# thuanz123/enhancing-transformers

Measured on AMD Instinct MI355X. Metric: images/sec ViT-VQGAN-base 256px stage-1 train; VQ argmin match-rate, higher is better.
Workload: dtype fp16; 1 GPU; imagenet_vitvq_base.yaml AE training step (1 fwd + 1 bwd + grad all-reduce + AdamW), loss = 1.0*L2 + 1.0*codebook (LPIPS/GAN weights 0), K=8192 x 32 l2-normalised codes, fp32 master weights, fp16 MFMA operands / fp32 accumulate, dynamic loss scale (now 65536; device-side inf/nan step skip + GradScaler update rule); per_gpu_batch=128, global_batch=128, image=256x256, parallelism=dp1, hip_graph_replay=False

## Files before the change

### enhancing-transformers_amd/csrc/common.h

```cpp
#pragma once
#include <hip/hip_runtime.h>
#include <stdint.h>
#include <stdio.h>
#include "../../include/enh_hip.h"

#define LDS_AS __attribute__((address_space(3)))
#define GLB_AS __attribute__((address_space(1)))
#ifdef ENH_GLDS_AUX_OVERRIDE
#define ENH_GLDS_AUX ENH_GLDS_AUX_OVERRIDE
#else
#define ENH_GLDS_AUX 0
#endif

typedef __attribute__((ext_vector_type(4))) float f32x4;
typedef __attribute__((ext_vector_type(4))) unsigned int u32x4;
typedef __attribute__((ext_vector_type(2))) unsigned int u32x2;
typedef __attribute__((ext_vector_type(16))) float f32x16;
typedef __attribute__((ext_vector_type(8))) __bf16 bf16x8;
typedef __attribute__((ext_vector_type(8))) short s16x8;
typedef __attribute__((ext_vector_type(4))) short s16x4;
typedef __attribute__((__vector_size__(4 * sizeof(__bf16)))) __bf16 bf16x4_t;

void enh_set_error(const char* fmt, ...);
int enh_check_launch(const char* what);
// ... 79 lines not shown
#define ENH_DT_DISPATCH(dtype, CALL)                    \
  do {                                                   \
    if ((dtype) == ENH_DT_F16) { typedef F16 OT; CALL; } \
    else { typedef BF16 OT; CALL; }                      \
  } while (0)
#define ENH_REQUIRE_DT(dtype, what) ENH_REQUIRE((dtype) == ENH_DT_BF16 || (dtype) == ENH_DT_F16, ENH_E_BADARG, what ": dtype must be ENH_DT_BF16 (0) or ENH_DT_F16 (1), got %d", (int)(dtype))

__device__ __forceinline__ float tanh_x3(float x) {
  const float x2 = x * x;
  const float t = __builtin_amdgcn_exp2f(x * 2.8853900817779268f);
  const float big = 1.f - 2.f * __builtin_amdgcn_rcpf(t + 1.f);
  const float small = x * (1.f + x2 * (-0.33333333333f + x2 * (0.13333333333f + x2 * -0.05396825397f)));
  return x2 < 0.0144f ? small : big;
}

__device__ inline s16x4 lds_tr_read_b64(const void* lds_ptr) {
  bf16x4_t v = __builtin_amdgcn_ds_read_tr16_b64_v4bf16((LDS_AS bf16x4_t*)lds_ptr);
  return __builtin_bit_cast(s16x4, v);
}

__device__ inline void lds_tr_read_b64_asm(unsigned long long& out, const void* lds_ptr) {
  const unsigned addr = (unsigned)(uintptr_t)(LDS_AS const void*)lds_ptr;
  asm volatile("ds_read_b64_tr_b16 %0, %1" : "=v"(out) : "v"(addr) : "memory");
}

__device__ inline float wave_sum(float v) {
#pragma unroll
  for (int o = 32; o > 0; o >>= 1) v += __shfl_xor(v, o, 64);
  return v;
}
__device__ inline float wave_max(float v) {
#pragma unroll
  for (int o = 32; o > 0; o >>= 1) v = fmaxf(v, __shfl_xor(v, o, 64));
  return v;
}

template <int NW, typename T>
__device__ __forceinline__ void block_publish(T wave_value, T* s_w) {
  static_assert(NW == 4 || NW == 16, "workgroups of 256 or 1024 threads");
  __syncthreads();
  if ((threadIdx.x & 63) == 0) s_w[threadIdx.x >> 6] = wave_value;
  __syncthreads();
}
template <int NW>
__device__ __forceinline__ float block_sum(float v, float* s_w) {
  block_publish<NW>(wave_sum(v), s_w);
  if constexpr (NW == 4) return ((s_w[0] + s_w[1]) + s_w[2]) + s_w[3];
  float s = 0.f;
#pragma unroll
  for (int i = 0; i < NW; ++i) s += s_w[i];
  return s;
}
template <int NW>
__device__ __forceinline__ float block_max(float v, float* s_w) {
  block_publish<NW>(wave_max(v), s_w);
  if constexpr (NW == 4) return fmaxf(fmaxf(s_w[0], s_w[1]), fmaxf(s_w[2], s_w[3]));
  float s = s_w[0];
#pragma unroll
  for (int i = 1; i < NW; ++i) s = fmaxf(s, s_w[i]);
  return s;
}
template <int NW>
__device__ __forceinline__ int block_count(int v, int* s_w) {
#pragma unroll
  for (int o = 32; o > 0; o >>= 1) v += __shfl_xor(v, o, 64);
  block_publish<NW>(v, s_w);
  int s = 0;
#pragma unroll
  for (int i = 0; i < NW; ++i) s += s_w[i];
  return s;
}

__device__ __forceinline__ u32x4 philox4x32_10(uint32_t k0, uint32_t k1, u32x4 c) {
#pragma unroll
  for (int r = 0; r < 10; ++r) {
    const uint32_t h0 = __umulhi(0xD2511F53u, c.x), l0 = 0xD2511F53u * c.x;
    const uint32_t h1 = __umulhi(0xCD9E8D57u, c.z), l1 = 0xCD9E8D57u * c.z;
    c = u32x4{h1 ^ c.y ^ k0, l1, h0 ^ c.w ^ k1, l0};
    k0 += 0x9E3779B9u; k1 += 0xBB67AE85u;
  }
  return c;
}

__device__ inline float fixed_order_rowsum16(const float* __restrict__ part, int rows, int64_t stride, int64_t n, bool n_ok, float* s_red ) {
  const int col = threadIdx.x & 15, grp = threadIdx.x >> 4;
  const int per = (rows + 15) / 16;
  const int r0 = grp * per, r1 = r0 + per < rows ? r0 + per : rows;
  float a = 0.f;
  if (n_ok)
    for (int r = r0; r < r1; ++r) a += part[(int64_t)r * stride + n];
  s_red[grp * 16 + col] = a;
  __syncthreads();
  float t = 0.f;
  if (grp == 0)
    for (int g = 0; g < 16; ++g) t += s_red[g * 16 + col];
  return t;
}
```

### enhancing-transformers_amd/csrc/elementwise.hip

```cpp
#include "common.h"

template <typename OT>
__global__ void patchify_kernel(const float* __restrict__ img, int B, int C, int H, int W, int p,
                                uint16_t* __restrict__ out, int64_t total4) {
  const int64_t i = (int64_t)blockIdx.x * blockDim.x + threadIdx.x;
  if (i >= total4) return;
  const int p4 = p >> 2, gx_n = W / p, gy_n = H / p;
  int64_t r = i;
  const int q = (int)(r % p4); r /= p4;
  const int ph = (int)(r % p); r /= p;
  const int c = (int)(r % C); r /= C;
  const int gx = (int)(r % gx_n);
  const int gy = (int)((r / gx_n) % gy_n);
  const int b = (int)(r / ((int64_t)gx_n * gy_n));
  const float4 v = *reinterpret_cast<const float4*>(img + (((size_t)b * C + c) * H + (size_t)gy * p + ph) * W + (size_t)gx * p + q * 4);
  *reinterpret_cast<uint2*>(out + (size_t)i * 4) = make_uint2(pack2<OT>(v.x, v.y), pack2<OT>(v.z, v.w));
}

template <typename OT>
__global__ __launch_bounds__(256) void unpatchify_loss_kernel(
    const float* __restrict__ pix, const float* __restrict__ target, int B, int C, int H, int W, int p, float w_l1,
    float w_l2, float inv_numel, float* __restrict__ xrec, double* __restrict__ sums, uint16_t* __restrict__ dpix,
    int64_t total4, const float* __restrict__ gscale) {
  __shared__ float s_l1[4], s_l2[4];
  if (gscale) inv_numel *= *gscale;
  const int64_t i = (int64_t)blockIdx.x * blockDim.x + threadIdx.x;
  float l1 = 0.f, l2 = 0.f;
  if (i < total4) {
    const int p4 = p >> 2, gx_n = W / p, gy_n = H / p;
    int64_t r = i;
    const int q = (int)(r % p4); r /= p4;
    const int ph = (int)(r % p); r /= p;
    const int c = (int)(r % C); r /= C;
    const int gx = (int)(r % gx_n);
    const int gy = (int)((r / gx_n) % gy_n);
    const int b = (int)(r / ((int64_t)gx_n * gy_n));
    const size_t off = (((size_t)b * C + c) * H + (size_t)gy * p + ph) * W + (size_t)gx * p + q * 4;
    const float4 v = *reinterpret_cast<const float4*>(pix + (size_t)i * 4);
    if (xrec) *reinterpret_cast<float4*>(xrec + off) = v;
    if (target) {
      const float4 x = *reinterpret_cast<const float4*>(target + off);
      const float d[4] = {v.x - x.x, v.y - x.y, v.z - x.z, v.w - x.w};
      float g[4];
#pragma unroll
      for (int k = 0; k < 4; ++k) {
        l1 += fabsf(d[k]);
        l2 += d[k] * d[k];
        const float sg = d[k] > 0.f ? 1.f : (d[k] < 0.f ? -1.f : 0.f);
        g[k] = (w_l1 * sg + w_l2 * 2.f * d[k]) * inv_numel;
      }
      if (dpix) *reinterpret_cast<uint2*>(dpix + (size_t)i * 4) = make_uint2(pack2<OT>(g[0], g[1]), pack2<OT>(g[2], g[3]));
    }
  }
  if (sums) {
    l1 = wave_sum(l1);
    l2 = wave_sum(l2);
    if ((threadIdx.x & 63) == 0) { s_l1[threadIdx.x >> 6] = l1; s_l2[threadIdx.x >> 6] = l2; }
    __syncthreads();
    if (threadIdx.x == 0) {
      atomicAdd(&sums[0], (double)((s_l1[0] + s_l1[1]) + (s_l1[2] + s_l1[3])));
      atomicAdd(&sums[1], (double)((s_l2[0] + s_l2[1]) + (s_l2[2] + s_l2[3])));
    }
  }
}

template <typename OT>
__global__ __launch_bounds__(256) void colsum_h16_kernel(const uint16_t* __restrict__ x, int64_t M, int64_t N,
                                                          int64_t ldx, int64_t rows_per_block, float* __restrict__ out, int64_t part_stride) {
  __shared__ float s_part[3][128];
  const int lane = threadIdx.x & 63, wave = threadIdx.x >> 6;
  const int64_t n0 = (int64_t)blockIdx.x * 128 + lane * 2;
  const int64_t m_begin = (int64_t)blockIdx.y * rows_per_block;
  int64_t m_end = m_begin + rows_per_block;
  if (m_end > M) m_end = M;
  float a0 = 0.f, a1 = 0.f;
  if (n0 < N) {
    for (int64_t m = m_begin + wave; m < m_end; m += 4) {
      const uint32_t u = *reinterpret_cast<const uint32_t*>(x + (size_t)m * ldx + n0);
      a0 += unpack_lo<OT>(u);
      a1 += unpack_hi<OT>(u);
    }
  }
  if (wave > 0) { s_part[wave - 1][lane * 2] = a0; s_part[wave - 1][lane * 2 + 1] = a1; }
  __syncthreads();
  if (wave == 0 && n0 < N) {
    for (int ww = 0; ww < 3; ++ww) { a0 += s_part[ww][lane * 2]; a1 += s_part[ww][lane * 2 + 1]; }
    { if (part_stride) out[(int64_t)blockIdx.y * part_stride + n0] = a0; else atomicAdd(&out[n0], a0); }
    { if (part_stride) out[(int64_t)blockIdx.y * part_stride + n0 + 1] = a1; else atomicAdd(&out[n0 + 1], a1); }
  }
}

template <typename OT>
__global__ __launch_bounds__(256) void colsum_h16_wide_kernel(const uint16_t* __restrict__ x, int64_t M, int64_t N, int64_t ldx,
                                                               int64_t rows_per_block, float* __restrict__ out, int64_t part_stride) {
  __shared__ float s_part[3][512];
  const int lane = threadIdx.x & 63, wave = threadIdx.x >> 6;
  const int64_t n0 = (int64_t)blockIdx.x * 512 + lane * 8;
  const int64_t m_begin = (int64_t)blockIdx.y * rows_per_block;
  int64_t m_end = m_begin + rows_per_block;
  if (m_end > M) m_end = M;
  float acc[8] = {0.f, 0.f, 0.f, 0.f, 0.f, 0.f, 0.f, 0.f};
  if (n0 < N) {
    const uint16_t* col = x + n0;
    int64_t m = m_begin + wave;
    for (; m + 12 < m_end; m += 16) {
      u32x4 v[4];
#pragma unroll
      for (int r = 0; r < 4; ++r) v[r] = *reinterpret_cast<const u32x4*>(col + (size_t)(m + 4 * r) * ldx);
#pragma unroll
      for (int r = 0; r < 4; ++r)
#pragma unroll
        for (int k = 0; k < 4; ++k) {
          acc[2 * k] += unpack_lo<OT>(v[r][k]);
          acc[2 * k + 1] += unpack_hi<OT>(v[r][k]);
        }
    }
    for (; m < m_end; m += 4) {
      const u32x4 v = *reinterpret_cast<const u32x4*>(col + (size_t)m * ldx);
#pragma unroll
      for (int k = 0; k < 4; ++k) {
        acc[2 * k] += unpack_lo<OT>(v[k]);
        acc[2 * k + 1] += unpack_hi<OT>(v[k]);
      }
    }
  }
  if (wave > 0) {
#pragma unroll
    for (int k = 0; k < 8; ++k) s_part[wave - 1][lane * 8 + k] = acc[k];
  }
  __syncthreads();
  if (wave == 0 && n0 < N) {
#pragma unroll
    for (int k = 0; k < 8; ++k) {
      float a = acc[k];
      for (int ww = 0; ww < 3; ++ww) a += s_part[ww][lane * 8 + k];
      { if (part_stride) out[(int64_t)blockIdx.y * part_stride + n0 + k] = a; else atomicAdd(&out[n0 + k], a); }
    }
  }
}

template <typename OT>
__global__ void cast_f32_h16_kernel(const float* __restrict__ x, uint16_t* __restrict__ y, int64_t n) {
  const int64_t i = ((int64_t)blockIdx.x * blockDim.x + threadIdx.x) * 4;
  if (i + 3 < n) {
    const float4 v = *reinterpret_cast<const float4*>(x + i);
    *reinterpret_cast<uint2*>(y + i) = make_uint2(pack2<OT>(v.x, v.y), pack2<OT>(v.z, v.w));
  } else {
    for (int64_t k = i; k < n; ++k) y[k] = pack1<OT>(x[k]);
  }
}

template <typename OT, bool CLIP>
__global__ void adamw_kernel(float* __restrict__ p, const float* __restrict__ g, float* __restrict__ m,
                             float* __restrict__ v, uint16_t* __restrict__ p16, int64_t n, float lr, float beta1,
                             float beta2, float eps, float wd, float gscale, float inv_bc1, float inv_sqrt_bc2, const float* __restrict__ skip,
                             const float* __restrict__ loss_scale, const float* __restrict__ clip_coef, float clip_value) {
  const int64_t i = ((int64_t)blockIdx.x * blockDim.x + threadIdx.x) * 4;
  if (i >= n) return;
  if (skip && *skip != 0.f) return;
  if (loss_scale) gscale /= *loss_scale;
  if (CLIP && clip_coef) gscale *= *clip_coef;
  float pv[4], gv[4], mv[4], vv[4];
  const bool full = i + 3 < n;
  if (full) {
    const float4 a = *reinterpret_cast<const float4*>(p + i), b = *reinterpret_cast<const float4*>(g + i);
    const float4 c = *reinterpret_cast<const float4*>(m + i), d = *reinterpret_cast<const float4*>(v + i);
    pv[0] = a.x; pv[1] = a.y; pv[2] = a.z; pv[3] = a.w; gv[0] = b.x; gv[1] = b.y; gv[2] = b.z; gv[3] = b.w;
    mv[0] = c.x; mv[1] = c.y; mv[2] = c.z; mv[3] = c.w; vv[0] = d.x; vv[1] = d.y; vv[2] = d.z; vv[3] = d.w;
  } else {
    for (int k = 0; k < 4; ++k) {
      const bool ok = i + k < n;
      pv[k] = ok ? p[i + k] : 0.f; gv[k] = ok ? g[i + k] : 0.f; mv[k] = ok ? m[i + k] : 0.f; vv[k] = ok ? v[i + k] : 0.f;
    }
  }
#pragma unroll
  for (int k = 0; k < 4; ++k) {
    float gg = gv[k] * gscale;
    if (CLIP && clip_value > 0.f) gg = gg > clip_value ? clip_value : (gg < -clip_value ? -clip_value : gg);
    pv[k] = pv[k] * (1.0f - lr * wd);
    mv[k] = mv[k] * beta1 + gg * (1.0f - beta1);
    vv[k] = vv[k] * beta2 + gg * gg * (1.0f - beta2);
    const float denom = sqrtf(vv[k]) * inv_sqrt_bc2 + eps;
    pv[k] = pv[k] - (lr * inv_bc1) * (mv[k] / denom);
  }
  if (full) {
    *reinterpret_cast<float4*>(p + i) = make_float4(pv[0], pv[1], pv[2], pv[3]);
    *reinterpret_cast<float4*>(m + i) = make_float4(mv[0], mv[1], mv[2], mv[3]);
    *reinterpret_cast<float4*>(v + i) = make_float4(vv[0], vv[1], vv[2], vv[3]);
    if (p16) *reinterpret_cast<uint2*>(p16 + i) = make_uint2(pack2<OT>(pv[0], pv[1]), pack2<OT>(pv[2], pv[3]));
  } else {
    for (int k = 0; k < 4 && i + k < n; ++k) {
      p[i + k] = pv[k]; m[i + k] = mv[k]; v[i + k] = vv[k];
      if (p16) p16[i + k] = pack1<OT>(pv[k]);
    }
  }
}

extern "C" int enh_patchify(const float* img, int B, int C, int H, int W, int p, enh_h16* patches, int dtype, void* stream) {
  ENH_REQUIRE_DT(dtype, "enh_patchify");
  ENH_REQUIRE(img && patches, ENH_E_BADARG, "enh_patchify: null pointer");
  ENH_REQUIRE(B > 0 && C > 0 && p > 0 && p % 4 == 0 && H % p == 0 && W % p == 0, ENH_E_SHAPE, "enh_patchify: need p %% 4 == 0 and H,W divisible by p (B=%d C=%d H=%d W=%d p=%d)", B, C, H, W, p);
  const int64_t total4 = (int64_t)B * C * H * W / 4;
  ENH_DT_DISPATCH(dtype, (patchify_kernel<OT><<<(int)((total4 + 255) / 256), 256, 0, (hipStream_t)stream>>>(img, B, C, H, W, p, patches, total4)));
  return enh_check_launch("enh_patchify");
}

extern "C" int enh_unpatchify_loss(const float* pix, const float* target, int B, int C, int H, int W, int p, float w_l1,
                                   float w_l2, float* xrec, double* sums, enh_h16* dpix_bf16, const float* grad_scale_dev, int dtype, void* stream) {
  ENH_REQUIRE_DT(dtype, "enh_unpatchify_loss");
  ENH_REQUIRE(pix && (xrec || target), ENH_E_BADARG, "enh_unpatchify_loss: null pointer");
  ENH_REQUIRE(B > 0 && C > 0 && p > 0 && p % 4 == 0 && H % p == 0 && W % p == 0, ENH_E_SHAPE, "enh_unpatchify_loss: need p %% 4 == 0 and H,W divisible by p");
  const int64_t numel = (int64_t)B * C * H * W, total4 = numel / 4;
  ENH_DT_DISPATCH(dtype, (unpatchify_loss_kernel<OT><<<(int)((total4 + 255) / 256), 256, 0, (hipStream_t)stream>>>(
      pix, target, B, C, H, W, p, w_l1, w_l2, 1.0f / (float)numel, xrec, target ? sums : nullptr, dpix_bf16, total4, grad_scale_dev)));
  return enh_check_launch("enh_unpatchify_loss");
}

__global__ __launch_bounds__(256) void colsum_reduce_kernel(const float* __restrict__ part, int chunks, int64_t N, float* __restrict__ out, int accumulate) {
  __shared__ float s_red[256];
  const int64_t n = (int64_t)blockIdx.x * 16 + (threadIdx.x & 15);
  const float t = fixed_order_rowsum16(part, chunks, N, n, n < N, s_red);
  if ((threadIdx.x >> 4) == 0 && n < N) out[n] = accumulate ? out[n] + t : t;
}

int enh_colsum_reduce_launch(const float* part, int chunks, int64_t N, float* out, int accumulate, hipStream_t s) {
  colsum_reduce_kernel<<<dim3((unsigned)((N + 15) / 16)), 256, 0, s>>>(part, chunks, N, out, accumulate);
  return enh_check_launch("colsum_reduce");
}

static int64_t colsum_chunks(int64_t M) {
  const int64_t chunks = (M + 511) / 512;
  return chunks > 256 ? 256 : chunks;
}

extern "C" size_t enh_colsum_h16_workspace_bytes(int64_t M, int64_t N) { return M > 0 && N > 0 ? (size_t)colsum_chunks(M) * N * sizeof(float) : 0; }

static int colsum_h16_impl(const enh_h16* x, int64_t M, int64_t N, int64_t ldx, float* out, int accumulate, float* part, int dtype, void* stream) {
  ENH_REQUIRE_DT(dtype, "enh_colsum_h16");
  ENH_REQUIRE(x && out, ENH_E_BADARG, "enh_colsum_h16: null pointer");
  ENH_REQUIRE(M > 0 && N > 0 && N % 2 == 0 && ldx % 2 == 0, ENH_E_SHAPE, "enh_colsum_h16: N and ldx must be even");
  hipStream_t s = (hipStream_t)stream;
  if (!accumulate && !part) {
    const int rc = enh_zero_f32_launch(out, N, s);
    if (rc) return rc;
  }
  const int64_t chunks = colsum_chunks(M);
  const int64_t rows_per_block = (M + chunks - 1) / chunks;
  float* dst = part ? part : out;
  const int64_t stride = part ? N : 0;
  if (N % 8 == 0 && ldx % 8 == 0 && ((uintptr_t)x & 15) == 0) {
    dim3 grid((unsigned)((N + 511) / 512), (unsigned)chunks);
    ENH_DT_DISPATCH(dtype, (colsum_h16_wide_kernel<OT><<<grid, 256, 0, s>>>(x, M, N, ldx, rows_per_block, dst, stride)));
  } else {
    dim3 grid((unsigned)((N + 127) / 128), (unsigned)chunks);
    ENH_DT_DISPATCH(dtype, (colsum_h16_kernel<OT><<<grid, 256, 0, s>>>(x, M, N, ldx, rows_per_block, dst, stride)));
  }
  if (part) colsum_reduce_kernel<<<dim3((unsigned)((N + 15) / 16)), 256, 0, s>>>(part, (int)chunks, N, out, accumulate);
  return enh_check_launch("enh_colsum_h16");
}

extern "C" int enh_colsum_h16(const enh_h16* x, int64_t M, int64_t N, int64_t ldx, float* out, int accumulate, int dtype, void* stream) {
  return colsum_h16_impl(x, M, N, ldx, out, accumulate, nullptr, dtype, stream);
}

extern "C" int enh_colsum_h16_ws(const enh_h16* x, int64_t M, int64_t N, int64_t ldx, float* out, int accumulate, void* ws, size_t ws_bytes, int dtype, void* stream) {
  ENH_REQUIRE(ws && ws_bytes >= enh_colsum_h16_workspace_bytes(M, N), ENH_E_WORKSPACE, "enh_colsum_h16_ws: workspace too small (%zu bytes)", ws_bytes);
  return colsum_h16_impl(x, M, N, ldx, out, accumulate, (float*)ws, dtype, stream);
}

template <typename OT>
__global__ void cast_f32_h16_head_scaled_kernel(const float* __restrict__ x, uint16_t* __restrict__ y, int64_t n, int64_t n_scaled, float alpha,
                                                 int64_t x_stride, int64_t y_stride) {
  x += (int64_t)blockIdx.y * x_stride; y += (int64_t)blockIdx.y * y_stride;
  const int64_t i = ((int64_t)blockIdx.x * blockDim.x + threadIdx.x) * 4;
  if (i >= n) return;
  if (i + 3 < n) {
    float4 v = *reinterpret_cast<const float4*>(x + i);
    if (i < n_scaled) { v.x *= alpha; v.y *= alpha; v.z *= alpha; v.w *= alpha; }
    *reinterpret_cast<uint2*>(y + i) = make_uint2(pack2<OT>(v.x, v.y), pack2<OT>(v.z, v.w));
  } else {
    for (int64_t k = i; k < n; ++k) y[k] = pack1<OT>(x[k] * (k < n_scaled ? alpha : 1.0f));
  }
}

extern "C" int enh_cast_f32_h16_head_scaled(const float* x, enh_h16* y, int64_t n, int64_t n_scaled, float alpha, int dtype, void* stream) {
  ENH_REQUIRE_DT(dtype, "enh_cast_f32_h16_head_scaled");
  ENH_REQUIRE(x && y && n > 0 && n_scaled >= 0 && n_scaled <= n && n_scaled % 4 == 0, ENH_E_BADARG, "enh_cast_f32_h16_head_scaled: bad argument");
  const int64_t n4 = (n + 3) / 4;
  ENH_DT_DISPATCH(dtype, (cast_f32_h16_head_scaled_kernel<OT><<<(int)((n4 + 255) / 256), 256, 0, (hipStream_t)stream>>>(x, y, n, n_scaled, alpha, 0, 0)));
  return enh_check_launch("enh_cast_f32_h16_head_scaled");
}

extern "C" int enh_cast_f32_h16_head_scaled_strided(const float* x, int64_t x_stride, enh_h16* y, int64_t y_stride, int64_t n, int64_t n_scaled, float alpha,
                                                     int count, int dtype, void* stream) {
  ENH_REQUIRE_DT(dtype, "enh_cast_f32_h16_head_scaled_strided");
  ENH_REQUIRE(x && y && n > 0 && n_scaled >= 0 && n_scaled <= n && n_scaled % 4 == 0 && count > 0 && count <= 65535, ENH_E_BADARG,
              "enh_cast_f32_h16_head_scaled_strided: bad argument");
  ENH_REQUIRE(x_stride % 4 == 0 && y_stride % 4 == 0 && y_stride >= n, ENH_E_SHAPE, "enh_cast_f32_h16_head_scaled_strided: strides must be multiples of 4 elements and the outputs disjoint");
  const int64_t n4 = (n + 3) / 4;
  ENH_DT_DISPATCH(dtype, (cast_f32_h16_head_scaled_kernel<OT><<<dim3((unsigned)((n4 + 255) / 256), (unsigned)count), 256, 0, (hipStream_t)stream>>>(x, y, n, n_scaled, alpha, x_stride, y_stride)));
  return enh_check_launch("enh_cast_f32_h16_head_scaled_strided");
}

extern "C" int enh_cast_f32_h16(const float* x, enh_h16* y, int64_t n, int dtype, void* stream) {
  ENH_REQUIRE_DT(dtype, "enh_cast_f32_h16");
  ENH_REQUIRE(x && y && n > 0, ENH_E_BADARG, "enh_cast_f32_h16: bad argument");
  const int64_t n4 = (n + 3) / 4;
  ENH_DT_DISPATCH(dtype, (cast_f32_h16_kernel<OT><<<(int)((n4 + 255) / 256), 256, 0, (hipStream_t)stream>>>(x, y, n)));
  return enh_check_launch("enh_cast_f32_h16");
}

extern "C" int enh_adamw_step(float* p, const float* g, float* m, float* v, enh_h16* p_bf16, int64_t n, int step,
                              float lr, float beta1, float beta2, float eps, float weight_decay, float grad_scale,
                              const float* skip_flag, const float* loss_scale_dev, const float* clip_coef_dev, float clip_value, int dtype,
                              void* stream) {
  ENH_REQUIRE_DT(dtype, "enh_adamw_step");
  ENH_REQUIRE(p && g && m && v && n > 0 && step >= 1 && clip_value >= 0.f, ENH_E_BADARG, "enh_adamw_step: bad argument");
  const double bc1 = 1.0 - pow((double)beta1, (double)step), bc2 = 1.0 - pow((double)beta2, (double)step);
  const int64_t n4 = (n + 3) / 4;
  const int grid = (int)((n4 + 255) / 256);
  const float inv_bc1 = (float)(1.0 / bc1), inv_sqrt_bc2 = (float)(1.0 / sqrt(bc2));
  if (clip_coef_dev || clip_value > 0.f)
    ENH_DT_DISPATCH(dtype, (adamw_kernel<OT, true><<<grid, 256, 0, (hipStream_t)stream>>>(p, g, m, v, p_bf16, n, lr, beta1, beta2, eps, weight_decay, grad_scale, inv_bc1,
                                                                                         inv_sqrt_bc2, skip_flag, loss_scale_dev, clip_coef_dev, clip_value)));
  else
    ENH_DT_DISPATCH(dtype, (adamw_kernel<OT, false><<<grid, 256, 0, (hipStream_t)stream>>>(p, g, m, v, p_bf16, n, lr, beta1, beta2, eps, weight_decay, grad_scale, inv_bc1,
                                                                                          inv_sqrt_bc2, skip_flag, loss_scale_dev, nullptr, 0.f)));
  return enh_check_launch("enh_adamw_step");
}

__global__ void loss_scale_update_kernel(float* __restrict__ scale, const float* __restrict__ found_inf, int* __restrict__ tracker, float growth, float backoff, int interval) {
  if (threadIdx.x != 0 || blockIdx.x != 0) return;
  float s = *scale;
  int t = *tracker;
  if (*found_inf != 0.f) { s *= backoff; t = 0; }
  else if (interval > 0 && ++t >= interval) { s *= growth; t = 0; }
  *scale = fminf(fmaxf(s, 1.0f), 16777216.0f);
  *tracker = t;
}

extern "C" int enh_loss_scale_update(float* scale, const float* found_inf, int* growth_tracker, float growth_factor, float backoff_factor, int growth_interval,
                                     void* stream) {
  ENH_REQUIRE(scale && found_inf && growth_tracker && growth_factor >= 1.f && backoff_factor > 0.f && backoff_factor <= 1.f && growth_interval >= 0, ENH_E_BADARG,
              "enh_loss_scale_update: bad argument (growth >= 1, 0 < backoff <= 1, interval >= 0)");
  loss_scale_update_kernel<<<1, 64, 0, (hipStream_t)stream>>>(scale, found_inf, growth_tracker, growth_factor, backoff_factor, growth_interval);
  return enh_check_launch("enh_loss_scale_update");
}

__global__ __launch_bounds__(256) void nonfinite_flag_kernel(const float* __restrict__ x, int64_t n, float* __restrict__ flag) {
  const int64_t stride = (int64_t)gridDim.x * blockDim.x * 4;
  const uint32_t* __restrict__ u = reinterpret_cast<const uint32_t*>(x);
  const int64_t n4 = n & ~(int64_t)3;
  uint32_t any = 0u;
  for (int64_t i = ((int64_t)blockIdx.x * blockDim.x + threadIdx.x) * 4; i < n4; i += stride) {
    const u32x4 v = *reinterpret_cast<const u32x4*>(u + i);
    const u32x4 e = (v >> 23) & 0xffu;
    any |= (uint32_t)(e[0] == 0xffu) | (uint32_t)(e[1] == 0xffu) | (uint32_t)(e[2] == 0xffu) | (uint32_t)(e[3] == 0xffu);
  }
  if (blockIdx.x == 0 && threadIdx.x < (unsigned)(n - n4)) any |= (uint32_t)(((u[n4 + threadIdx.x] >> 23) & 0xffu) == 0xffu);
  if (__builtin_amdgcn_ballot_w64(any != 0u) != 0 && (threadIdx.x & 63) == 0) *flag = 1.0f;
}

extern "C" int enh_nonfinite_flag(const float* x, int64_t n, float* flag, void* stream) {
  ENH_REQUIRE(x && flag && n > 0 && ((uintptr_t)x & 15) == 0, ENH_E_BADARG, "enh_nonfinite_flag: bad argument (x 16-byte aligned)");
  const int64_t n4 = (n + 3) / 4;
  const int64_t want = (n4 + 255) / 256;
  const int grid = (int)(want < 2048 ? want : 2048);
  nonfinite_flag_kernel<<<grid, 256, 0, (hipStream_t)stream>>>(x, n, flag);
  return enh_check_launch("enh_nonfinite_flag");
}

__device__ __forceinline__ double block_sum_f64_fixed(double a, double* s_wave) {
#pragma unroll
  for (int off = 32; off > 0; off >>= 1) a += __shfl_xor(a, off, 64);
  if ((threadIdx.x & 63) == 0) s_wave[threadIdx.x >> 6] = a;
  __syncthreads();
  return ((s_wave[0] + s_wave[1]) + s_wave[2]) + s_wave[3];
}

__global__ __launch_bounds__(256) void grad_sumsq_kernel(const float* __restrict__ x, int64_t n, double* __restrict__ part, float* __restrict__ flag) {
  __shared__ double s_wave[4];
  const int64_t stride = (int64_t)gridDim.x * blockDim.x * 4;
  const uint32_t* __restrict__ u = reinterpret_cast<const uint32_t*>(x);
  const int64_t n4 = n & ~(int64_t)3;
  uint32_t any = 0u;
  double acc = 0.0;
  for (int64_t i = ((int64_t)blockIdx.x * blockDim.x + threadIdx.x) * 4; i < n4; i += stride) {
    const u32x4 v = *reinterpret_cast<const u32x4*>(u + i);
    const u32x4 e = (v >> 23) & 0xffu;
    any |= (uint32_t)(e[0] == 0xffu) | (uint32_t)(e[1] == 0xffu) | (uint32_t)(e[2] == 0xffu) | (uint32_t)(e[3] == 0xffu);
    const float a = __uint_as_float(v[0]), b = __uint_as_float(v[1]), c = __uint_as_float(v[2]), d = __uint_as_float(v[3]);
    acc += (double)((a * a + b * b) + (c * c + d * d));
  }
  if (blockIdx.x == 0 && threadIdx.x < (unsigned)(n - n4)) {
    const uint32_t t = u[n4 + threadIdx.x];
    any |= (uint32_t)(((t >> 23) & 0xffu) == 0xffu);
    const float a = __uint_as_float(t);
    acc += (double)(a * a);
  }
  if (flag && __builtin_amdgcn_ballot_w64(any != 0u) != 0 && (threadIdx.x & 63) == 0) *flag = 1.0f;
  const double t = block_sum_f64_fixed(acc, s_wave);
  if (threadIdx.x == 0) part[blockIdx.x] = t;
}

__global__ __launch_bounds__(256) void grad_clip_finish_kernel(const double* __restrict__ part, int parts, float max_norm, float grad_scale,
                                                               const float* __restrict__ loss_scale, float* __restrict__ out) {
  __shared__ double s_wave[4];
  double acc = 0.0;
  for (int i = threadIdx.x; i < parts; i += 256) acc += part[i];
  const double sum = block_sum_f64_fixed(acc, s_wave);
  if (threadIdx.x != 0) return;
  const double total = sqrt(sum) * (double)grad_scale / (loss_scale ? (double)*loss_scale : 1.0);
  const double c = (double)max_norm / (total + 1e-6);
  out[0] = (float)total;
  out[1] = (float)(c > 1.0 ? 1.0 : c);
}

static int grad_sumsq_grid(int64_t n) {
  const int64_t n4 = (n + 3) / 4;
  const int64_t want = (n4 + 255) / 256;
  return (int)(want < 2048 ? want : 2048);
}

extern "C" size_t enh_grad_clip_coef_workspace_bytes(int64_t n) { return n > 0 ? (size_t)grad_sumsq_grid(n) * sizeof(double) : 0; }

extern "C" int enh_grad_clip_coef(const float* g, int64_t n, float max_norm, float grad_scale, const float* loss_scale_dev, float* found_inf, float* out,
                                  void* ws, size_t ws_bytes, void* stream) {
  ENH_REQUIRE(g && out && n > 0 && ((uintptr_t)g & 15) == 0 && !(max_norm < 0.f) && max_norm == max_norm, ENH_E_BADARG,
              "enh_grad_clip_coef: bad argument (g 16-byte aligned, max_norm >= 0)");
  ENH_REQUIRE(ws && ((uintptr_t)ws & 7) == 0 && ws_bytes >= enh_grad_clip_coef_workspace_bytes(n), ENH_E_WORKSPACE,
              "enh_grad_clip_coef: workspace too small or misaligned (%zu bytes)", ws_bytes);
  const int grid = grad_sumsq_grid(n);
  grad_sumsq_kernel<<<grid, 256, 0, (hipStream_t)stream>>>(g, n, (double*)ws, found_inf);
  grad_clip_finish_kernel<<<1, 256, 0, (hipStream_t)stream>>>((const double*)ws, grid, max_norm, grad_scale, loss_scale_dev, out);
  return enh_check_launch("enh_grad_clip_coef");
}

__global__ __launch_bounds__(256) void crop_flip_u8_kernel(const uint8_t* __restrict__ src, const int* __restrict__ meta, float* __restrict__ out, int B, int Hs,
                                                           int Ws, int R) {
  const int64_t idx = (int64_t)blockIdx.x * blockDim.x + threadIdx.x;
  const int64_t total = (int64_t)B * R * R;
  if (idx >= total) return;
  const int x = (int)(idx % R), y = (int)((idx / R) % R);
  const int64_t b = idx / ((int64_t)R * R);
  const int y0 = meta[b * 3 + 0], x0 = meta[b * 3 + 1], flip = meta[b * 3 + 2];
  const int sx = x0 + (flip ? R - 1 - x : x), sy = y0 + y;
  const uint8_t* p = src + ((b * Hs + sy) * (int64_t)Ws + sx) * 3;
  float* o = out + b * 3 * (int64_t)R * R + (int64_t)y * R + x;
  o[0] = (float)p[0] / 255.0f;
  o[(int64_t)R * R] = (float)p[1] / 255.0f;
  o[2 * (int64_t)R * R] = (float)p[2] / 255.0f;
}

extern "C" int enh_crop_flip_u8(const uint8_t* src, int B, int Hs, int Ws, const int32_t* meta, int R, float* out, void* stream) {
  ENH_REQUIRE(src && meta && out && B > 0 && R > 0 && Hs >= R && Ws >= R, ENH_E_BADARG, "enh_crop_flip_u8: bad argument (the staging slot must hold an R x R window)");
  const int64_t total = (int64_t)B * R * R;
  crop_flip_u8_kernel<<<dim3((unsigned)((total + 255) / 256)), 256, 0, (hipStream_t)stream>>>(src, meta, out, B, Hs, Ws, R);
  return enh_check_launch("enh_crop_flip_u8");
}
```

### enhancing-transformers_amd/csrc/layernorm.hip

```cpp
#include "common.h"

template <int NCH, bool X3, typename OT>
__global__ __launch_bounds__(256) void ln_fwd_kernel(const float* __restrict__ x, const float* __restrict__ w,
                                                     const float* __restrict__ b, int64_t M, int D, float eps,
                                                     uint16_t* __restrict__ y16, float* __restrict__ y32,
                                                     float* __restrict__ mean_out, float* __restrict__ rstd_out, uint16_t* __restrict__ y3) {
  const int lane = threadIdx.x & 63;
  const int64_t row = (int64_t)blockIdx.x * 4 + (threadIdx.x >> 6);
  if (row >= M) return;
  const int nch = D >> 2;
  const float4* xr = reinterpret_cast<const float4*>(x + (size_t)row * D);
  float4 v[NCH];
  float s = 0.f;
#pragma unroll
  for (int i = 0; i < NCH; ++i) {
    const int c = lane + 64 * i;
    v[i] = c < nch ? xr[c] : make_float4(0.f, 0.f, 0.f, 0.f);
    s += (v[i].x + v[i].y) + (v[i].z + v[i].w);
  }
  const float mean = wave_sum(s) / (float)D;
  float q = 0.f;
#pragma unroll
  for (int i = 0; i < NCH; ++i) {
    const int c = lane + 64 * i;
// ... 151 lines not shown
            part[((size_t)blockIdx.x * 3 + 0) * D + c * 4 + k] = aw[k];
            part[((size_t)blockIdx.x * 3 + 1) * D + c * 4 + k] = ab[k];
          } else {
            atomicAdd(&dw[c * 4 + k], aw[k]);
            atomicAdd(&db[c * 4 + k], ab[k]);
          }
        }
      }
    }
  }
  if (dxsum) {
    __syncthreads();
    if (wave > 0) {
#pragma unroll
      for (int i = 0; i < NCH; ++i) {
        float* pw = &s_dw[wave - 1][(lane + 64 * i) * 4];
        pw[0] = adx[i].x; pw[1] = adx[i].y; pw[2] = adx[i].z; pw[3] = adx[i].w;
      }
    }
    __syncthreads();
    if (wave == 0) {
#pragma unroll
      for (int i = 0; i < NCH; ++i) {
        const int c = lane + 64 * i;
        if (c < nch) {
          float ax[4] = {adx[i].x, adx[i].y, adx[i].z, adx[i].w};
#pragma unroll
          for (int k = 0; k < 4; ++k) {
            for (int ww = 0; ww < 3; ++ww) ax[k] += s_dw[ww][c * 4 + k];
            if (part) part[((size_t)blockIdx.x * 3 + 2) * D + c * 4 + k] = ax[k];
            else atomicAdd(&dxsum[c * 4 + k], ax[k]);
          }
        }
      }
    }
  }
}

template <bool X3, typename OT>
static void ln_fwd_launch(int grid, hipStream_t s, const float* x, const float* w, const float* b, int64_t M, int D, float eps, enh_h16* y_bf16, float* y_f32,
                          float* mean, float* rstd, enh_h16* y3) {
  switch ((D + 255) / 256) {
    case 1: ln_fwd_kernel<1, X3, OT><<<grid, 256, 0, s>>>(x, w, b, M, D, eps, y_bf16, y_f32, mean, rstd, y3); break;
    case 2: ln_fwd_kernel<2, X3, OT><<<grid, 256, 0, s>>>(x, w, b, M, D, eps, y_bf16, y_f32, mean, rstd, y3); break;
    case 3: ln_fwd_kernel<3, X3, OT><<<grid, 256, 0, s>>>(x, w, b, M, D, eps, y_bf16, y_f32, mean, rstd, y3); break;
    case 4: ln_fwd_kernel<4, X3, OT><<<grid, 256, 0, s>>>(x, w, b, M, D, eps, y_bf16, y_f32, mean, rstd, y3); break;
    case 5: ln_fwd_kernel<5, X3, OT><<<grid, 256, 0, s>>>(x, w, b, M, D, eps, y_bf16, y_f32, mean, rstd, y3); break;
    default: ln_fwd_kernel<8, X3, OT><<<grid, 256, 0, s>>>(x, w, b, M, D, eps, y_bf16, y_f32, mean, rstd, y3); break;
  }
}

extern "C" int enh_layernorm_forward(const float* x, const float* w, const float* b, int64_t M, int D, float eps,
                                     enh_h16* y_bf16, float* y_f32, float* mean, float* rstd, int dtype, void* stream) {
  ENH_REQUIRE_DT(dtype, "enh_layernorm_forward");
  ENH_REQUIRE(x && w && b && (y_bf16 || y_f32), ENH_E_BADARG, "enh_layernorm_forward: null pointer");
  ENH_REQUIRE(M > 0 && D > 0 && D % 4 == 0 && D <= 2048, ENH_E_SHAPE, "enh_layernorm_forward: need D %% 4 == 0 and D <= 2048, got M=%lld D=%d", (long long)M, D);
  ENH_DT_DISPATCH(dtype, (ln_fwd_launch<false, OT>((int)((M + 3) / 4), (hipStream_t)stream, x, w, b, M, D, eps, y_bf16, y_f32, mean, rstd, nullptr)));
  return enh_check_launch("enh_layernorm_forward");
}

extern "C" int enh_layernorm_forward_x3(const float* x, const float* w, const float* b, int64_t M, int D, float eps, enh_h16* y3,
                                        enh_h16* y_bf16, float* y_f32, float* mean, float* rstd, void* stream) {
  ENH_REQUIRE(x && w && b && y3, ENH_E_BADARG, "enh_layernorm_forward_x3: null pointer");
  ENH_REQUIRE(M > 0 && D > 0 && D % 4 == 0 && D <= 2048, ENH_E_SHAPE, "enh_layernorm_forward_x3: need D %% 4 == 0 and D <= 2048, got M=%lld D=%d", (long long)M, D);
  ln_fwd_launch<true, BF16>((int)((M + 3) / 4), (hipStream_t)stream, x, w, b, M, D, eps, y_bf16, y_f32, mean, rstd, y3);
  return enh_check_launch("enh_layernorm_forward_x3");
}

template <bool DY16, typename OT>
static void ln_bwd_launch(int grid, hipStream_t s, const void* dy, const float* x, const float* w, const float* mean, const float* rstd,
                          const float* dres, int64_t M, int D, float* dx_f32, enh_h16* dx_bf16, float* dw, float* db, float* dx_colsum, float* part) {
  switch ((D + 255) / 256) {
    case 1: ln_bwd_kernel<1, DY16, OT><<<grid, 256, 0, s>>>(dy, x, w, mean, rstd, dres, M, D, dx_f32, dx_bf16, dw, db, dx_colsum, part); break;
    case 2: ln_bwd_kernel<2, DY16, OT><<<grid, 256, 0, s>>>(dy, x, w, mean, rstd, dres, M, D, dx_f32, dx_bf16, dw, db, dx_colsum, part); break;
    case 3: ln_bwd_kernel<3, DY16, OT><<<grid, 256, 0, s>>>(dy, x, w, mean, rstd, dres, M, D, dx_f32, dx_bf16, dw, db, dx_colsum, part); break;
    case 4: ln_bwd_kernel<4, DY16, OT><<<grid, 256, 0, s>>>(dy, x, w, mean, rstd, dres, M, D, dx_f32, dx_bf16, dw, db, dx_colsum, part); break;
    case 5: ln_bwd_kernel<5, DY16, OT><<<grid, 256, 0, s>>>(dy, x, w, mean, rstd, dres, M, D, dx_f32, dx_bf16, dw, db, dx_colsum, part); break;
    default: ln_bwd_kernel<8, DY16, OT><<<grid, 256, 0, s>>>(dy, x, w, mean, rstd, dres, M, D, dx_f32, dx_bf16, dw, db, dx_colsum, part); break;
  }
}

__global__ __launch_bounds__(256) void ln_bwd_reduce_kernel(const float* __restrict__ part, int nwg, int D, float* __restrict__ dw, float* __restrict__ db,
                                                            float* __restrict__ dxsum) {
  __shared__ float s_red[256];
  const int which = blockIdx.y;
  float* out = which == 0 ? dw : (which == 1 ? db : dxsum);
  if (!out) return;
  const int j = blockIdx.x * 16 + (threadIdx.x & 15);
  const float t = fixed_order_rowsum16(part + (size_t)which * D, nwg, (int64_t)3 * D, j, j < D, s_red);
  if ((threadIdx.x >> 4) == 0 && j < D) out[j] += t;
}

static int ln_bwd_grid(int64_t M, bool for_workspace = false) {
  const int64_t want = (M + 3) / 4;
  const int cus = for_workspace ? enh_device_cus() : enh_cu_budget();
  return (int)(want < cus ? want : cus);
}

extern "C" size_t enh_layernorm_backward_workspace_bytes(int64_t M, int D) {
  return M > 0 && D > 0 ? (size_t)ln_bwd_grid(M, true) * 3 * D * sizeof(float) : 0;
}

static int ln_bwd_impl(const float* dy, const enh_h16* dy_bf16, const float* x, const float* w, const float* mean, const float* rstd, const float* dres,
                       int64_t M, int D, float* dx_f32, enh_h16* dx_bf16, float* dw, float* db, float* dx_colsum, float* part, int dtype, void* stream) {
  ENH_REQUIRE_DT(dtype, "enh_layernorm_backward");
  ENH_REQUIRE((dy != nullptr) != (dy_bf16 != nullptr), ENH_E_BADARG, "enh_layernorm_backward: pass exactly one of dy (f32) / dy_bf16");
  ENH_REQUIRE(x && w && mean && rstd && dx_f32 && dw && db, ENH_E_BADARG, "enh_layernorm_backward: null pointer");
  ENH_REQUIRE(M > 0 && D > 0 && D % 4 == 0 && D <= 2048, ENH_E_SHAPE, "enh_layernorm_backward: need D %% 4 == 0 and D <= 2048, got M=%lld D=%d", (long long)M, D);
  hipStream_t s = (hipStream_t)stream;
  const int grid = ln_bwd_grid(M);
  if (dy_bf16) ENH_DT_DISPATCH(dtype, (ln_bwd_launch<true, OT>(grid, s, dy_bf16, x, w, mean, rstd, dres, M, D, dx_f32, dx_bf16, dw, db, dx_colsum, part)));
  else ENH_DT_DISPATCH(dtype, (ln_bwd_launch<false, OT>(grid, s, dy, x, w, mean, rstd, dres, M, D, dx_f32, dx_bf16, dw, db, dx_colsum, part)));
  if (part) ln_bwd_reduce_kernel<<<dim3((unsigned)((D + 15) / 16), 3), 256, 0, s>>>(part, grid, D, dw, db, dx_colsum);
  return enh_check_launch("enh_layernorm_backward");
}

extern "C" int enh_layernorm_backward(const float* dy, const enh_h16* dy_bf16, const float* x, const float* w, const float* mean,
                                      const float* rstd, const float* dres, int64_t M, int D, float* dx_f32,
                                      enh_h16* dx_bf16, float* dw, float* db, float* dx_colsum, int dtype, void* stream) {
  return ln_bwd_impl(dy, dy_bf16, x, w, mean, rstd, dres, M, D, dx_f32, dx_bf16, dw, db, dx_colsum, nullptr, dtype, stream);
}

extern "C" int enh_layernorm_backward_ws(const float* dy, const enh_h16* dy_bf16, const float* x, const float* w, const float* mean,
                                         const float* rstd, const float* dres, int64_t M, int D, float* dx_f32,
                                         enh_h16* dx_bf16, float* dw, float* db, float* dx_colsum, void* ws, size_t ws_bytes, int dtype, void* stream) {
  ENH_REQUIRE(ws && ws_bytes >= enh_layernorm_backward_workspace_bytes(M, D), ENH_E_WORKSPACE, "enh_layernorm_backward_ws: workspace too small (%zu bytes)", ws_bytes);
  return ln_bwd_impl(dy, dy_bf16, x, w, mean, rstd, dres, M, D, dx_f32, dx_bf16, dw, db, dx_colsum, (float*)ws, dtype, stream);
}
```

Baseline: 623.2 images/s.

## Stage unpatchify loss through LDS tiles and widen fixed-order column reductions

The unpatchify+loss kernel now processes tiles in a grid-stride loop. Each tile's patch tokens are loaded coalesced into LDS and then read back in image order, so the reads of pix, the writes of xrec and dpix, and the reads of target are all contiguous rather than scattered. Per-thread loss partials accumulate in double precision across tiles. The fixed-order row-sum used by colsum and layernorm-backward reductions now handles two adjacent columns per thread with float2 loads and an 8-deep unrolled loop, which halves the number of reduction workgroups. These changes add LDS traffic and barriers, and they cap the grid at three blocks per CU, which could limit occupancy on this small loss kernel.

```diff
diff --git a/enhancing-transformers_amd/csrc/common.h b/enhancing-transformers_amd/csrc/common.h
--- a/enhancing-transformers_amd/csrc/common.h
+++ b/enhancing-transformers_amd/csrc/common.h
@@ -185,17 +185,38 @@
   return c;
 }
 
-__device__ inline float fixed_order_rowsum16(const float* __restrict__ part, int rows, int64_t stride, int64_t n, bool n_ok, float* s_red ) {
-  const int col = threadIdx.x & 15, grp = threadIdx.x >> 4;
+__device__ inline float fixed_order_rowsum16(const float* __restrict__ part, int rows, int64_t stride, int64_t n0, int64_t N, float* s_red ) {
+  const int pair = threadIdx.x & 15, grp = threadIdx.x >> 4;
   const int per = (rows + 15) / 16;
   const int r0 = grp * per, r1 = r0 + per < rows ? r0 + per : rows;
-  float a = 0.f;
-  if (n_ok)
-    for (int r = r0; r < r1; ++r) a += part[(int64_t)r * stride + n];
-  s_red[grp * 16 + col] = a;
+  const int64_t n = n0 + 2 * pair;
+  const float* __restrict__ p = part + (int64_t)r0 * stride + n;
+  float a0 = 0.f, a1 = 0.f;
+  if (n + 1 < N && (stride & 1) == 0 && ((uintptr_t)part & 7) == 0) {
+    int r = r0;
+    for (; r + 8 <= r1; r += 8, p += 8 * stride) {
+      float2 v[8];
+#pragma unroll
+      for (int k = 0; k < 8; ++k) v[k] = *reinterpret_cast<const float2*>(p + k * stride);
+#pragma unroll
+      for (int k = 0; k < 8; ++k) { a0 += v[k].x; a1 += v[k].y; }
+    }
+    for (; r < r1; ++r, p += stride) {
+      const float2 v = *reinterpret_cast<const float2*>(p);
+      a0 += v.x; a1 += v.y;
+    }
+  } else if (n < N) {
+    const bool two = n + 1 < N;
+    for (int r = r0; r < r1; ++r, p += stride) {
+      a0 += p[0];
+      if (two) a1 += p[1];
+    }
+  }
+  s_red[grp * 32 + 2 * pair] = a0;
+  s_red[grp * 32 + 2 * pair + 1] = a1;
   __syncthreads();
   float t = 0.f;
-  if (grp == 0)
-    for (int g = 0; g < 16; ++g) t += s_red[g * 16 + col];
+  if (threadIdx.x < 32)
+    for (int g = 0; g < 16; ++g) t += s_red[g * 32 + threadIdx.x];
   return t;
 }
diff --git a/enhancing-transformers_amd/csrc/elementwise.hip b/enhancing-transformers_amd/csrc/elementwise.hip
--- a/enhancing-transformers_amd/csrc/elementwise.hip
+++ b/enhancing-transformers_amd/csrc/elementwise.hip
@@ -17,49 +17,119 @@
   *reinterpret_cast<uint2*>(out + (size_t)i * 4) = make_uint2(pack2<OT>(v.x, v.y), pack2<OT>(v.z, v.w));
 }
 
+__device__ __forceinline__ double block_sum_f64_fixed(double a, double* s_wave) {
+#pragma unroll
+  for (int off = 32; off > 0; off >>= 1) a += __shfl_xor(a, off, 64);
+  if ((threadIdx.x & 63) == 0) s_wave[threadIdx.x >> 6] = a;
+  __syncthreads();
+  return ((s_wave[0] + s_wave[1]) + s_wave[2]) + s_wave[3];
+}
+
+constexpr int UNP_TILE_F4 = 1024;
+constexpr int UNP_LDS_FLOATS = 5120;
+constexpr int UNP_TERMS_F32 = 16;
 template <typename OT>
 __global__ __launch_bounds__(256) void unpatchify_loss_kernel(
-    const float* __restrict__ pix, const float* __restrict__ target, int B, int C, int H, int W, int p, float w_l1,
+    const float* __restrict__ pix, const float* __restrict__ target, int C, int H, int W, int p, float w_l1,
     float w_l2, float inv_numel, float* __restrict__ xrec, double* __restrict__ sums, uint16_t* __restrict__ dpix,
-    int64_t total4, const float* __restrict__ gscale) {
-  __shared__ float s_l1[4], s_l2[4];
+    int cpt, int gxt, int tiles, const float* __restrict__ gscale) {
+  __shared__ __attribute__((aligned(16))) float s_tile[UNP_LDS_FLOATS];
+  __shared__ double s_w1[4], s_w2[4];
+  static_assert(UNP_TERMS_F32 == 4 * (UNP_TILE_F4 / 256), "a thread's share of a tile: UNP_TILE_F4 / 256 float4 of four terms");
   if (gscale) inv_numel *= *gscale;
-  const int64_t i = (int64_t)blockIdx.x * blockDim.x + threadIdx.x;
-  float l1 = 0.f, l2 = 0.f;
-  if (i < total4) {
-    const int p4 = p >> 2, gx_n = W / p, gy_n = H / p;
-    int64_t r = i;
-    const int q = (int)(r % p4); r /= p4;
-    const int ph = (int)(r % p); r /= p;
-    const int c = (int)(r % C); r /= C;
-    const int gx = (int)(r % gx_n);
-    const int gy = (int)((r / gx_n) % gy_n);
-    const int b = (int)(r / ((int64_t)gx_n * gy_n));
-    const size_t off = (((size_t)b * C + c) * H + (size_t)gy * p + ph) * W + (size_t)gx * p + q * 4;
-    const float4 v = *reinterpret_cast<const float4*>(pix + (size_t)i * 4);
-    if (xrec) *reinterpret_cast<float4*>(xrec + off) = v;
-    if (target) {
-      const float4 x = *reinterpret_cast<const float4*>(target + off);
-      const float d[4] = {v.x - x.x, v.y - x.y, v.z - x.z, v.w - x.w};
-      float g[4];
+  const unsigned tid = threadIdx.x;
+  const unsigned up = (unsigned)p, p4 = up >> 2, gx_n = (unsigned)(W / p), gy_n = (unsigned)(H / p), cp_n = (unsigned)(C * p);
+  const unsigned n_cpt = (cp_n + cpt - 1) / cpt, n_gxt = (gx_n + gxt - 1) / gxt;
+  const size_t cpp = (size_t)cp_n * up;
+  double l1d = 0.0, l2d = 0.0;
+  for (unsigned tile = blockIdx.x; tile < (unsigned)tiles; tile += gridDim.x) {
+    unsigned r = tile;
+    const unsigned cp0 = (r % n_cpt) * cpt; r /= n_cpt;
+    const unsigned gx0 = (r % n_gxt) * gxt; r /= n_gxt;
+    const unsigned gy = r % gy_n, b = r / gy_n;
+    const unsigned cpt_c = cp_n - cp0 < (unsigned)cpt ? cp_n - cp0 : (unsigned)cpt, gxt_c = gx_n - gx0 < (unsigned)gxt ? gx_n - gx0 : (unsigned)gxt;
+    const unsigned run = cpt_c * up, run4 = run >> 2;
+    const unsigned ts = run + ((up - run) & 63u);
+    const unsigned n4 = gxt_c * run4;
+    const size_t tok0 = (((size_t)b * gy_n + gy) * gx_n + gx0) * cpp + (size_t)cp0 * up;
+    const size_t img0 = ((size_t)b * C * H + (size_t)gy * up) * W + (size_t)gx0 * up;
+    unsigned la_t[4];
+    size_t off_t[4];
+    float4 v[4];
+    {
+      unsigned g = tid / run4, w = tid - g * run4;
+      const unsigned ig = 256u / run4, iw = 256u - ig * run4;
 #pragma unroll
       for (int k = 0; k < 4; ++k) {
-        l1 += fabsf(d[k]);
-        l2 += d[k] * d[k];
-        const float sg = d[k] > 0.f ? 1.f : (d[k] < 0.f ? -1.f : 0.f);
-        g[k] = (w_l1 * sg + w_l2 * 2.f * d[k]) * inv_numel;
+        la_t[k] = g * ts + w * 4;
+        off_t[k] = tok0 + (size_t)g * cpp + w * 4;
+        v[k] = tid + 256u * k < n4 ? *reinterpret_cast<const float4*>(pix + off_t[k]) : make_float4(0.f, 0.f, 0.f, 0.f);
+        w += iw; g += ig;
+        if (w >= run4) { w -= run4; ++g; }
       }
-      if (dpix) *reinterpret_cast<uint2*>(dpix + (size_t)i * 4) = make_uint2(pack2<OT>(g[0], g[1]), pack2<OT>(g[2], g[3]));
+    }
+    unsigned la_i[4];
+    size_t off_i[4];
+    float4 x[4];
+    {
+      unsigned t = tid / p4, q = tid - t * p4;
+      unsigned rr = t / gxt_c, g = t - rr * gxt_c;
+      unsigned c = (cp0 + rr) / up, ph = (cp0 + rr) - c * up;
+      const unsigned it = 256u / p4, iq = 256u - it * p4;
+      const unsigned ir = it / gxt_c, ig = it - ir * gxt_c;
+      const unsigned ic = ir / up, iph = ir - ic * up;
+#pragma unroll
+      for (int k = 0; k < 4; ++k) {
+        la_i[k] = g * ts + rr * up + q * 4;
+        off_i[k] = img0 + ((size_t)c * H + ph) * W + g * up + q * 4;
+        x[k] = tid + 256u * k < n4 && target ? *reinterpret_cast<const float4*>(target + off_i[k]) : make_float4(0.f, 0.f, 0.f, 0.f);
+        q += iq; g += ig; rr += ir; ph += iph; c += ic;
+        if (q >= p4) { q -= p4; ++g; }
+        if (g >= gxt_c) { g -= gxt_c; ++rr; ++ph; }
+        if (ph >= up) { ph -= up; ++c; }
+      }
+    }
+    __syncthreads();
+#pragma unroll
+    for (int k = 0; k < 4; ++k)
+      if (tid + 256u * k < n4) *reinterpret_cast<float4*>(&s_tile[la_t[k]]) = v[k];
+    __syncthreads();
+    float l1 = 0.f, l2 = 0.f;
+#pragma unroll
+    for (int e = 0; e < 4; ++e) {
+      if (tid + 256u * e >= n4) break;
+      const float4 vi = *reinterpret_cast<const float4*>(&s_tile[la_i[e]]);
+      if (xrec) *reinterpret_cast<float4*>(xrec + off_i[e]) = vi;
+      if (target) {
+        const float d[4] = {vi.x - x[e].x, vi.y - x[e].y, vi.z - x[e].z, vi.w - x[e].w};
+        float g[4];
+#pragma unroll
+        for (int k = 0; k < 4; ++k) {
+          l1 += fabsf(d[k]);
+          l2 += d[k] * d[k];
+          const float sg = d[k] > 0.f ? 1.f : (d[k] < 0.f ? -1.f : 0.f);
+          g[k] = (w_l1 * sg + w_l2 * 2.f * d[k]) * inv_numel;
+        }
+        if (dpix) *reinterpret_cast<float4*>(&s_tile[la_i[e]]) = make_float4(g[0], g[1], g[2], g[3]);
+      }
+    }
+    l1d += (double)l1;
+    l2d += (double)l2;
+    if (target && dpix) {
+      __syncthreads();
+#pragma unroll
+      for (int k = 0; k < 4; ++k)
+        if (tid + 256u * k < n4) {
+          const float4 g = *reinterpret_cast<const float4*>(&s_tile[la_t[k]]);
+          *reinterpret_cast<uint2*>(dpix + off_t[k]) = make_uint2(pack2<OT>(g.x, g.y), pack2<OT>(g.z, g.w));
+        }
     }
   }
   if (sums) {
-    l1 = wave_sum(l1);
-    l2 = wave_sum(l2);
-    if ((threadIdx.x & 63) == 0) { s_l1[threadIdx.x >> 6] = l1; s_l2[threadIdx.x >> 6] = l2; }
-    __syncthreads();
-    if (threadIdx.x == 0) {
-      atomicAdd(&sums[0], (double)((s_l1[0] + s_l1[1]) + (s_l1[2] + s_l1[3])));
-      atomicAdd(&sums[1], (double)((s_l2[0] + s_l2[1]) + (s_l2[2] + s_l2[3])));
+    const double t1 = block_sum_f64_fixed(l1d, s_w1), t2 = block_sum_f64_fixed(l2d, s_w2);
+    if (tid == 0) {
+      atomicAdd(&sums[0], t1);
+      atomicAdd(&sums[1], t2);
     }
   }
 }
@@ -210,21 +280,33 @@
   ENH_REQUIRE_DT(dtype, "enh_unpatchify_loss");
   ENH_REQUIRE(pix && (xrec || target), ENH_E_BADARG, "enh_unpatchify_loss: null pointer");
   ENH_REQUIRE(B > 0 && C > 0 && p > 0 && p % 4 == 0 && H % p == 0 && W % p == 0, ENH_E_SHAPE, "enh_unpatchify_loss: need p %% 4 == 0 and H,W divisible by p");
-  const int64_t numel = (int64_t)B * C * H * W, total4 = numel / 4;
-  ENH_DT_DISPATCH(dtype, (unpatchify_loss_kernel<OT><<<(int)((total4 + 255) / 256), 256, 0, (hipStream_t)stream>>>(
-      pix, target, B, C, H, W, p, w_l1, w_l2, 1.0f / (float)numel, xrec, target ? sums : nullptr, dpix_bf16, total4, grad_scale_dev)));
+  ENH_REQUIRE(p <= 4 * UNP_TILE_F4 && (int64_t)C * p < (1 << 24), ENH_E_SHAPE, "enh_unpatchify_loss: patch size %d (x %d channels) beyond the tile of the kernel", p, C);
+  const int64_t numel = (int64_t)B * C * H * W;
+  const int cp_n = C * p, gx_n = W / p;
+  const int cpt = cp_n < 4 * UNP_TILE_F4 / p ? cp_n : 4 * UNP_TILE_F4 / p;
+  const int run = cpt * p;
+  int gxt_max = 4 * UNP_TILE_F4 / run < UNP_LDS_FLOATS / (run + 60) ? 4 * UNP_TILE_F4 / run : UNP_LDS_FLOATS / (run + 60);
+  if (gxt_max > gx_n) gxt_max = gx_n;
+  const int n_gxt = (gx_n + gxt_max - 1) / gxt_max, gxt = (gx_n + n_gxt - 1) / n_gxt;
+  const int64_t tiles = (int64_t)B * (H / p) * ((gx_n + gxt - 1) / gxt) * ((cp_n + cpt - 1) / cpt);
+  ENH_REQUIRE(tiles < ((int64_t)1 << 31), ENH_E_SHAPE, "enh_unpatchify_loss: too many tiles (%lld)", (long long)tiles);
+  const int64_t cap = (int64_t)3 * enh_device_cus();
+  const int grid = (int)(tiles < cap ? tiles : cap);
+  ENH_DT_DISPATCH(dtype, (unpatchify_loss_kernel<OT><<<grid, 256, 0, (hipStream_t)stream>>>(
+      pix, target, C, H, W, p, w_l1, w_l2, 1.0f / (float)numel, xrec, target ? sums : nullptr, dpix_bf16, cpt, gxt, (int)tiles, grad_scale_dev)));
   return enh_check_launch("enh_unpatchify_loss");
 }
 
 __global__ __launch_bounds__(256) void colsum_reduce_kernel(const float* __restrict__ part, int chunks, int64_t N, float* __restrict__ out, int accumulate) {
-  __shared__ float s_red[256];
-  const int64_t n = (int64_t)blockIdx.x * 16 + (threadIdx.x & 15);
-  const float t = fixed_order_rowsum16(part, chunks, N, n, n < N, s_red);
-  if ((threadIdx.x >> 4) == 0 && n < N) out[n] = accumulate ? out[n] + t : t;
+  __shared__ float s_red[512];
+  const int64_t n0 = (int64_t)blockIdx.x * 32;
+  const float t = fixed_order_rowsum16(part, chunks, N, n0, N, s_red);
+  const int64_t n = n0 + threadIdx.x;
+  if (threadIdx.x < 32 && n < N) out[n] = accumulate ? out[n] + t : t;
 }
 
 int enh_colsum_reduce_launch(const float* part, int chunks, int64_t N, float* out, int accumulate, hipStream_t s) {
-  colsum_reduce_kernel<<<dim3((unsigned)((N + 15) / 16)), 256, 0, s>>>(part, chunks, N, out, accumulate);
+  colsum_reduce_kernel<<<dim3((unsigned)((N + 31) / 32)), 256, 0, s>>>(part, chunks, N, out, accumulate);
   return enh_check_launch("colsum_reduce");
 }
 
@@ -255,7 +337,7 @@
     dim3 grid((unsigned)((N + 127) / 128), (unsigned)chunks);
     ENH_DT_DISPATCH(dtype, (colsum_h16_kernel<OT><<<grid, 256, 0, s>>>(x, M, N, ldx, rows_per_block, dst, stride)));
   }
-  if (part) colsum_reduce_kernel<<<dim3((unsigned)((N + 15) / 16)), 256, 0, s>>>(part, (int)chunks, N, out, accumulate);
+  if (part) return enh_colsum_reduce_launch(part, (int)chunks, N, out, accumulate, s);
   return enh_check_launch("enh_colsum_h16");
 }
 
@@ -370,13 +452,6 @@
   return enh_check_launch("enh_nonfinite_flag");
 }
 
-__device__ __forceinline__ double block_sum_f64_fixed(double a, double* s_wave) {
-#pragma unroll
-  for (int off = 32; off > 0; off >>= 1) a += __shfl_xor(a, off, 64);
-  if ((threadIdx.x & 63) == 0) s_wave[threadIdx.x >> 6] = a;
-  __syncthreads();
-  return ((s_wave[0] + s_wave[1]) + s_wave[2]) + s_wave[3];
-}
 
 __global__ __launch_bounds__(256) void grad_sumsq_kernel(const float* __restrict__ x, int64_t n, double* __restrict__ part, float* __restrict__ flag) {
   __shared__ double s_wave[4];
diff --git a/enhancing-transformers_amd/csrc/layernorm.hip b/enhancing-transformers_amd/csrc/layernorm.hip
--- a/enhancing-transformers_amd/csrc/layernorm.hip
+++ b/enhancing-transformers_amd/csrc/layernorm.hip
@@ -257,13 +257,14 @@
 
 __global__ __launch_bounds__(256) void ln_bwd_reduce_kernel(const float* __restrict__ part, int nwg, int D, float* __restrict__ dw, float* __restrict__ db,
                                                             float* __restrict__ dxsum) {
-  __shared__ float s_red[256];
+  __shared__ float s_red[512];
   const int which = blockIdx.y;
   float* out = which == 0 ? dw : (which == 1 ? db : dxsum);
   if (!out) return;
-  const int j = blockIdx.x * 16 + (threadIdx.x & 15);
-  const float t = fixed_order_rowsum16(part + (size_t)which * D, nwg, (int64_t)3 * D, j, j < D, s_red);
-  if ((threadIdx.x >> 4) == 0 && j < D) out[j] += t;
+  const int j0 = blockIdx.x * 32;
+  const float t = fixed_order_rowsum16(part + (size_t)which * D, nwg, (int64_t)3 * D, j0, D, s_red);
+  const int j = j0 + threadIdx.x;
+  if (threadIdx.x < 32 && j < D) out[j] += t;
 }
 
 static int ln_bwd_grid(int64_t M, bool for_workspace = false) {
@@ -286,7 +287,7 @@
   const int grid = ln_bwd_grid(M);
   if (dy_bf16) ENH_DT_DISPATCH(dtype, (ln_bwd_launch<true, OT>(grid, s, dy_bf16, x, w, mean, rstd, dres, M, D, dx_f32, dx_bf16, dw, db, dx_colsum, part)));
   else ENH_DT_DISPATCH(dtype, (ln_bwd_launch<false, OT>(grid, s, dy, x, w, mean, rstd, dres, M, D, dx_f32, dx_bf16, dw, db, dx_colsum, part)));
-  if (part) ln_bwd_reduce_kernel<<<dim3((unsigned)((D + 15) / 16), 3), 256, 0, s>>>(part, grid, D, dw, db, dx_colsum);
+  if (part) ln_bwd_reduce_kernel<<<dim3((unsigned)((D + 31) / 32), 3), 256, 0, s>>>(part, grid, D, dw, db, dx_colsum);
   return enh_check_launch("enh_layernorm_backward");
 }
 
```

Measured after the change: 627.0 images/s, median of 6. Within noise of the previous version (+0.6%).
